# ZpokenWeb3/zk-light-client-implementation

Measured on AMD Instinct MI355X. Metric: Block_i BFT-finality proofs/sec (100 validators), higher is better.
Workload: dtype u64

## Files before the change

### __graft_entry__.py

```python
import os
import subprocess
import sys

ROOT = os.path.dirname(os.path.abspath(__file__))
if ROOT not in sys.path:
    sys.path.insert(0, ROOT)


def build() -> None:
    import concurrent.futures
    import importlib
    b = importlib.import_module("zk-light-client-implementation_amd.build")
    pool = concurrent.futures.ThreadPoolExecutor(max_workers=1)
    devsim = pool.submit(b.build_devsim, True)
    b.build(verbose=True)
    mk = os.path.join(ROOT, "oracle", "c", "Makefile")
    if os.path.exists(mk):
        subprocess.check_call(["make", "-s", "-C", os.path.dirname(mk)])
    import zklc_amd
    zklc_amd.load()
    lib_dir = os.path.join(ROOT, "zk-light-client-implementation_amd", "lib")
    subprocess.check_call(["gcc", "-O2", "-Wall", "-Wextra", "-std=c11", "-D_POSIX_C_SOURCE=200809L", "-I", os.path.join(ROOT, "include"),
                           os.path.join(ROOT, "tests", "c_abi", "prove_from_file.c"), "-o", os.path.join(ROOT, "tests", "c_abi", "prove_from_file"),
                           "-L", lib_dir, "-lzklc_mi355", "-Wl,-rpath,$ORIGIN/../../zk-light-client-implementation_amd/lib"])
    b.build_poseidon_gate_dev(True)
    devsim.result()
    pool.shutdown()


def smoke() -> None:
    import json
    import numpy as np
    import zklc_amd
    from oracle import ed25519_ref as ref

    with zklc_amd.Context(0) as ctx:
        j = json.load(open(os.path.join(ROOT, "tests", "golden", "ed25519_near_c1_small.json")))
        msg = bytes.fromhex(j["msg"])
        pks = b"".join(bytes.fromhex(e["validator_tail"])[1:33] for e in j["entries"])
        sigs = b"".join(bytes.fromhex(e["approval"])[2:] for e in j["entries"])
        ok = ctx.ed25519_verify_batch(pks, sigs, msg)
        exp = [int(ref.verify(pks[32 * i:32 * i + 32], sigs[64 * i:64 * i + 64], msg)) for i in range(len(ok))]
        assert ok.tolist() == exp == [1, 1, 1], (ok.tolist(), exp)
        m2 = b"zklc smoke"
        pk2, sg2, exp2 = [], [], []
        for i in range(64):
            sd = ref.synthetic_seed(11, i)
            _, _, pk = ref.keypair(sd)
            s = bytearray(ref.sign(sd, m2))
            if i % 5 == 4:
                s[i % 64] ^= 0x10
            pk2.append(pk)
            sg2.append(bytes(s))
            exp2.append(int(ref.verify(pk, bytes(s), m2)))
        ok2 = ctx.ed25519_verify_batch(b"".join(pk2), b"".join(sg2), m2)
        assert ok2.tolist() == exp2, "GPU Ed25519 batch differs from the oracle"
        assert sum(exp2) == 64 - 12
        from zklc_amd.plonky2 import CircuitBuilder, serialization as S, HASH_GL
        from oracle import plonky2_prover as OP, plonky2_verifier as V
        b = CircuitBuilder()
        x = b.add_virtual_public_input()
        y = b.add_virtual_target()
        z = b.mul(x, y)
        b.split_le(x, 10)
        lo, hi = b.mul_add_u32(x, y, b.constant(77))
        b.register_public_input(lo)
        b.connect(b.sub(b.add(z, b.constant(5)), z), b.constant(5))
        data = b.build()
        wires, pis = data.generate_witness({x: 1000, y: 4000000000})
        prover = data.prover(ctx, HASH_GL)
        raw = prover.prove_bytes(wires, pis)
        common = data.common_data()
        oproof, ovd = OP.prove(common, data.constants, data.sigmas, wires, pis, V.HasherGL)
        assert raw == S.proof_to_bytes(oproof, common, HASH_GL), "GPU plonky2 proof differs from the oracle prover"
        V.verify(json.loads(json.dumps(S.proof_from_bytes(raw, common, HASH_GL))), prover.verifier_data(), common)
        from zklc_amd.plonky2.recursion import RecursionProver
        rp = RecursionProver(ctx, HASH_GL)
        rc, rproof = rp.recursive_proof((common, prover.verifier_data(), raw), None, [7, 8])
        V.verify(json.loads(json.dumps(rproof)), rc.verifier_only, rc.common)
        assert rproof["public_inputs"] == [7, 8]
        bad = bytearray(raw)
        bad[800] ^= 1
        try:
            rp.recursive_proof((common, prover.verifier_data(), bytes(bad)), None, [7, 8])
            raise SystemExit("smoke: a tampered inner proof was accepted by the in-circuit verifier")
        except AssertionError:
            pass
        rp.close()
        prover.close()
    print("smoke OK: Ed25519 batch verify, a plonky2 proof and a recursive proof on cuda:0 match the oracle")


if __name__ == "__main__":
    build()
    if "--smoke" in sys.argv:
        smoke()
```

### zk-light-client-implementation_amd/build.py

```python
import concurrent.futures as cf
import glob
import os
import subprocess
import sys

HERE = os.path.dirname(os.path.abspath(__file__))
CSRC = os.path.join(HERE, "csrc")
BUILD = os.path.join(HERE, "build")
LIBDIR = os.path.join(HERE, "lib")
LIB = os.path.join(LIBDIR, "libzklc_mi355.so")
HIPCC = os.environ.get("HIPCC", "/opt/rocm/bin/hipcc")
FLAGS = ["--offload-arch=gfx950", "-O3", "-std=c++17", "-fPIC", "-fno-gpu-rdc", "-Wall", "-Wno-unused-function"]


def _newest(paths):
    return max((os.path.getmtime(p) for p in paths), default=0.0)


HOST_CXX = os.environ.get("CXX", "g++")
HOST_FLAGS = ["-O3", "-funroll-loops", "-std=c++17", "-fPIC", "-pthread", "-Wall", "-Wno-unused-function", "-Wno-unknown-pragmas"]


def _compile(src, obj, log):
    cmd = ([HIPCC] + FLAGS if src.endswith(".hip") else [HOST_CXX] + HOST_FLAGS) + ["-c", src, "-o", obj]
    r = subprocess.run(cmd, capture_output=True, text=True)
    if r.returncode != 0:
        raise RuntimeError("hipcc failed for %s:\n%s\n%s" % (src, r.stdout, r.stderr))
    if log:
        print("[zklc build] compiled", os.path.basename(src), file=sys.stderr)
    return obj


def build(verbose=True, force=False):
    os.makedirs(BUILD, exist_ok=True)
    os.makedirs(LIBDIR, exist_ok=True)
    srcs = sorted(glob.glob(os.path.join(CSRC, "*.hip")) + glob.glob(os.path.join(CSRC, "*.cpp")))
    hdrs = glob.glob(os.path.join(CSRC, "*.cuh")) + glob.glob(os.path.join(CSRC, "*.h")) + glob.glob(
        os.path.join(CSRC, "*.inc")) + glob.glob(os.path.join(HERE, "..", "include", "*.h"))
    dep_time = _newest(hdrs + [os.path.abspath(__file__)])
    jobs, objs = [], []
    for s in srcs:
        o = os.path.join(BUILD, os.path.basename(s).replace(".", "_") + ".o")
        objs.append(o)
        if force or not os.path.exists(o) or os.path.getmtime(o) < max(os.path.getmtime(s), dep_time):
            jobs.append((s, o))
    if jobs:
        with cf.ThreadPoolExecutor(max_workers=min(len(jobs), os.cpu_count() or 4)) as ex:
            list(ex.map(lambda so: _compile(so[0], so[1], verbose), jobs))
    if jobs or not os.path.exists(LIB) or os.path.getmtime(LIB) < _newest(objs):
        cmd = [HIPCC, "--offload-arch=gfx950", "-shared", "-fPIC", "-pthread", "-o", LIB] + objs
        r = subprocess.run(cmd, capture_output=True, text=True)
        if r.returncode != 0:
            raise RuntimeError("link failed:\n%s\n%s" % (r.stdout, r.stderr))
        if verbose:
            print("[zklc build] linked", LIB, file=sys.stderr)
    return LIB


DEVSIM_DIR = os.path.join(HERE, "..", "tests", "devsim")
DEVSIM_SRC = os.path.join(DEVSIM_DIR, "devsim.hip")
DEVSIM_LIB = os.path.join(DEVSIM_DIR, "libdevsim.so")


def devsim_sources():
    return [DEVSIM_SRC, os.path.abspath(__file__)] + [p for ext in ("*.cuh", "*.h", "*.inc") for p in glob.glob(os.path.join(CSRC, ext))]


def devsim_is_current():
    return os.path.exists(DEVSIM_LIB) and os.path.getmtime(DEVSIM_LIB) >= _newest(devsim_sources())


def build_devsim(verbose=True, force=False):
    if force or not devsim_is_current():
        r = subprocess.run([HIPCC] + FLAGS + ["-shared", DEVSIM_SRC, "-o", DEVSIM_LIB], capture_output=True, text=True)
        if r.returncode != 0:
            raise RuntimeError("hipcc failed for %s:\n%s\n%s" % (DEVSIM_SRC, r.stdout, r.stderr))
        if verbose:
            print("[zklc build] built", DEVSIM_LIB, file=sys.stderr)
    return DEVSIM_LIB


PGD_DIR = os.path.join(HERE, "..", "tests", "poseidon_gate_dev")
PGD_SRC = os.path.join(PGD_DIR, "poseidon_gate_dev.hip")
PGD_LIB = os.path.join(PGD_DIR, "libposeidon_gate_dev.so")


def poseidon_gate_dev_is_current():
    deps = [PGD_SRC, os.path.abspath(__file__)] + [p for ext in ("*.cuh", "*.h", "*.inc") for p in glob.glob(os.path.join(CSRC, ext))]
    return os.path.exists(PGD_LIB) and os.path.getmtime(PGD_LIB) >= _newest(deps)


def build_poseidon_gate_dev(verbose=True, force=False):
    if force or not poseidon_gate_dev_is_current():
        r = subprocess.run([HIPCC] + FLAGS + ["-Wno-inline-asm", "-shared", PGD_SRC, "-o", PGD_LIB], capture_output=True, text=True)
        if r.returncode != 0:
            raise RuntimeError("hipcc failed for %s:\n%s\n%s" % (PGD_SRC, r.stdout, r.stderr))
        if verbose:
            print("[zklc build] built", PGD_LIB, file=sys.stderr)
    return PGD_LIB


if __name__ == "__main__":
    build(force="--force" in sys.argv)
    build_devsim(force="--force" in sys.argv)
    build_poseidon_gate_dev(force="--force" in sys.argv)
```

### zk-light-client-implementation_amd/csrc/plonky2_prover.hip

```cpp
#include <algorithm>
#include <chrono>
#include <stdio.h>
#include <stdlib.h>
#include <new>
#include <vector>
#include <string.h>
#include "plonky2_gates.cuh"
#include "plonky2_host.h"
#include "plonky2_perm_terms.cuh"
#include "zklc_internal.h"

#define P2_THREADS 256

struct p2_challenges {
    u64 beta[P2_MAX_CH], gamma[P2_MAX_CH], alpha[P2_MAX_CH];
};

__global__ void p2_pow_table_kernel(u64 *out, u64 base, u64 n) {
    u64 i = (u64)blockIdx.x * blockDim.x + threadIdx.x;
    if (i < n) out[i] = gl_pow(base, i);
}

__global__ void p2_scale_by_powers_kernel(u64 *data, u64 base, u64 n) {
    u64 j = (u64)blockIdx.x * blockDim.x + threadIdx.x;
    if (j >= n) return;
    u64 *p = data + (size_t)blockIdx.y * n + j;
    *p = gl_mul(*p, gl_pow(base, j));
}

#define P2_SCALE_PER_LANE 8
__global__ void __launch_bounds__(256) p2_scale_by_powers_strided_kernel(u64 *data, u64 base, u64 step, u64 n) {
    const u64 j0 = (u64)blockIdx.x * (256 * P2_SCALE_PER_LANE) + threadIdx.x;
    if (j0 >= n) return;
    u64 *p = data + (size_t)blockIdx.y * n;
    u64 v[P2_SCALE_PER_LANE];
#pragma unroll
    for (int q = 0; q < P2_SCALE_PER_LANE; q++) v[q] = j0 + 256 * q < n ? p[j0 + 256 * q] : 0;
    u64 pw = gl_pow(base, j0);
#pragma unroll
    for (int q = 0; q < P2_SCALE_PER_LANE; q++) {
        if (j0 + 256 * q < n) p[j0 + 256 * q] = gl_mul(v[q], pw);
        if (q + 1 < P2_SCALE_PER_LANE) pw = gl_mul(pw, step);
    }
}

__global__ void p2_ext_powers_kernel(gl2 *out, gl2 z, u64 n) {
    u64 j = (u64)blockIdx.x * blockDim.x + threadIdx.x;
    if (j < n) out[j] = gl2_pow(z, j);
}

__global__ void p2_ext_pow_limbs_kernel(u32 *out, gl2 z, u32 n) {
    u32 j = blockIdx.x * blockDim.x + threadIdx.x;
    if (j >= n) return;
    gl2 v = gl2_pow(z, j);
    gl_limbs22(v.a, out + 12 * (size_t)j);
    gl_limbs22(v.b, out + 12 * (size_t)j + 6);
}

template <bool LEAN>
__global__ void __launch_bounds__(P2_THREADS)
p2_chunk_products_kernel(const u64 *__restrict__ wires, const u64 *__restrict__ sigmas, const u64 *__restrict__ subgroup,
                         const u64 *__restrict__ k_is, u32 n, u32 routed, u32 qdf, u32 nchunks, u64 beta, u64 gamma,
                         u64 *__restrict__ rp) {
    u32 i = blockIdx.x * blockDim.x + threadIdx.x;
    if (i >= n) return;
    u64 x = subgroup[i];
    u64 nums[16], dens[16];
    for (u32 k = 0; k < nchunks; k++) {
        u64 np = 1, dp = 1;
        u32 end = (k + 1) * qdf < routed ? (k + 1) * qdf : routed;
        if constexpr (LEAN) {
            const u64 bx = gl_mul(beta, x);
            for (u32 j = k * qdf; j < end; j += P2_PERM_CHUNK) {
                const u32 cnt = end - j < P2_PERM_CHUNK ? end - j : P2_PERM_CHUNK;
                u64 wv[P2_PERM_CHUNK], sv[P2_PERM_CHUNK], kv[P2_PERM_CHUNK], n8, d8;
#pragma unroll
                for (u32 q = 0; q < P2_PERM_CHUNK; q++) {
                    const u32 jq = q < cnt ? j + q : j;
                    wv[q] = wires[(size_t)jq * n + i];
                    sv[q] = sigmas[(size_t)jq * n + i];
                    kv[q] = k_is[jq];
                }
                p2_perm_chunk_terms(wv, sv, kv, cnt, beta, bx, gamma, n8, d8);
                if (j == k * qdf) {
                    np = n8;
                    dp = d8;
                } else {
                    np = gl_mul(np, n8);
                    dp = gl_mul(dp, d8);
                }
            }
        } else {
// ... 708 lines not shown
}

#define P2_EVAL_SPLIT 8
__global__ void __launch_bounds__(P2_THREADS)
p2_eval_at_ext_kernel(const u64 *__restrict__ coeffs, u32 n, const gl2 *__restrict__ zpow, const u64 *__restrict__ scale,
                      gl2 *__restrict__ partial) {
    __shared__ gl2 sh[P2_THREADS];
    const u64 *c = coeffs + (size_t)blockIdx.x * n;
    u32 slice = (n + P2_EVAL_SPLIT - 1) / P2_EVAL_SPLIT;
    u32 j0 = blockIdx.y * slice, j1 = j0 + slice < n ? j0 + slice : n;
    gl2 acc = gl2_make(0, 0);
    u32 j = j0 + threadIdx.x;
    for (; j + 3 * P2_THREADS < j1; j += 4 * P2_THREADS) {
        u64 c0 = c[j], c1 = c[j + P2_THREADS], c2 = c[j + 2 * P2_THREADS], c3 = c[j + 3 * P2_THREADS];
        gl2 z0 = zpow[j], z1 = zpow[j + P2_THREADS], z2 = zpow[j + 2 * P2_THREADS], z3 = zpow[j + 3 * P2_THREADS];
        if (scale) {
            c0 = gl_mul(c0, scale[j]);
            c1 = gl_mul(c1, scale[j + P2_THREADS]);
            c2 = gl_mul(c2, scale[j + 2 * P2_THREADS]);
            c3 = gl_mul(c3, scale[j + 3 * P2_THREADS]);
        }
        acc = gl2_add(acc, gl2_add(gl2_add(gl2_scale(z0, c0), gl2_scale(z1, c1)), gl2_add(gl2_scale(z2, c2), gl2_scale(z3, c3))));
    }
    for (; j < j1; j += P2_THREADS) {
        u64 cj = c[j];
        if (scale) cj = gl_mul(cj, scale[j]);
        acc = gl2_add(acc, gl2_scale(zpow[j], cj));
    }
    sh[threadIdx.x] = acc;
    __syncthreads();
    for (u32 off = P2_THREADS / 2; off; off >>= 1) {
        if (threadIdx.x < off) sh[threadIdx.x] = gl2_add(sh[threadIdx.x], sh[threadIdx.x + off]);
        __syncthreads();
    }
    if (threadIdx.x == 0) partial[(size_t)blockIdx.x * P2_EVAL_SPLIT + blockIdx.y] = sh[0];
}
__global__ void p2_eval_finish_kernel(const gl2 *__restrict__ partial, u32 n_polys, gl2 *__restrict__ out) {
    u32 b = blockIdx.x * blockDim.x + threadIdx.x;
    if (b >= n_polys) return;
    gl2 acc = partial[(size_t)b * P2_EVAL_SPLIT];
    for (u32 s = 1; s < P2_EVAL_SPLIT; s++) acc = gl2_add(acc, partial[(size_t)b * P2_EVAL_SPLIT + s]);
    out[b] = acc;
}

struct p2_fri_combine_args {
    const u64 *mats[4];
    u32 widths[4];
    u32 lde_bits, nch;
    u64 w_lde;
    gl2 alpha, zeta, g_zeta, y0, y1, alpha_pow_nch;
    gl2 *out;
    const u32 *apow;
    const u64 *xs;
};
__global__ void __launch_bounds__(P2_THREADS) p2_fri_denominators_kernel(const u64 *__restrict__ xs, u32 lde_bits, gl2 zeta, gl2 g_zeta,
                                                                           gl2 *__restrict__ out) {
    const size_t N = (size_t)1 << lde_bits;
    const size_t p0 = ((size_t)blockIdx.x * blockDim.x + threadIdx.x) * P2_FRI_DEN_POINTS;
    if (p0 >= N) return;
    u64 x[P2_FRI_DEN_POINTS];
    gl2 r[P2_FRI_DEN_POINTS];
#pragma unroll
    for (int q = 0; q < P2_FRI_DEN_POINTS; q++) x[q] = p0 + q < N ? xs[p0 + q] : 0;
    p2_fri_den_inverse_norms(x, zeta, g_zeta, r);
#pragma unroll
    for (int q = 0; q < P2_FRI_DEN_POINTS; q++)
        if (p0 + q < N) out[p0 + q] = r[q];
}
template <bool LEAN>
__global__ void __launch_bounds__(P2_THREADS) p2_fri_combine_kernel(p2_fri_combine_args a) {
    const size_t N = (size_t)1 << a.lde_bits;
    size_t p = (size_t)blockIdx.x * blockDim.x + threadIdx.x;
    if (p >= N) return;
    u64 x;
    [[maybe_unused]] gl2 ninv = gl2_make(0, 0);
    if constexpr (LEAN) {
        x = a.xs[p];
        ninv = a.out[p];
    } else {
        u64 i = __brevll((u64)p) >> (64 - a.lde_bits);
        x = gl_mul(GL_GENERATOR, gl_pow(a.w_lde, i));
    }
    gl_acc3 sa = {0, 0, 0}, sb = {0, 0, 0};
    gl_ktab *k6 = (gl_ktab *)a.apow;
    u32 terms = 0;
    for (int m = 0; m < 4; m++) {
        const u64 *mat = a.mats[m] + p;
        const u32 w = a.widths[m];
        u32 j = 0;
        for (; j + 16 <= w; j += 16, k6 += 16 * 12) {
            u64 v[16];
#pragma unroll
            for (int q = 0; q < 16; q++) v[q] = mat[(size_t)(j + q) * N];
#pragma unroll
            for (int q = 0; q < 16; q++) {
                gl_acc3_mul(sa, v[q], k6 + 12 * q);
                gl_acc3_mul(sb, v[q], k6 + 12 * q + 6);
            }
            if ((terms += 16) >= 384) {
                terms = 0;
                gl_acc3_normalize(sa);
                gl_acc3_normalize(sb);
            }
        }
        for (; j < w; j++, k6 += 12) {
            u64 v = mat[(size_t)j * N];
            gl_acc3_mul(sa, v, k6);
            gl_acc3_mul(sb, v, k6 + 6);
        }
        terms += 16;
    }
    gl2 acc = gl2_make(gl_acc3_reduce(sa), gl_acc3_reduce(sb));
    gl_acc3 ta = {0, 0, 0}, tb = {0, 0, 0};
    for (u32 j = 0; j < a.nch; j++) {
        u64 v = a.mats[2][(size_t)j * N + p];
        gl_acc3_mul(ta, v, (gl_ktab *)a.apow + 12 * (size_t)j);
        gl_acc3_mul(tb, v, (gl_ktab *)a.apow + 12 * (size_t)j + 6);
    }
    gl2 acc1 = gl2_make(gl_acc3_reduce(ta), gl_acc3_reduce(tb));
    gl2 i0, i1;
    if constexpr (LEAN) {
        i0 = p2_fri_den_inverse(x, a.zeta, ninv.a);
        i1 = p2_fri_den_inverse(x, a.g_zeta, ninv.b);
    } else {
        i0 = gl2_inv(gl2_sub(gl2_make(x, 0), a.zeta));
        i1 = gl2_inv(gl2_sub(gl2_make(x, 0), a.g_zeta));
    }
    gl2 q0 = gl2_mul(gl2_sub(acc, a.y0), i0);
    gl2 q1 = gl2_mul(gl2_sub(acc1, a.y1), i1);
    a.out[p] = gl2_add(gl2_mul(q0, a.alpha_pow_nch), q1);
}

__global__ void __launch_bounds__(P2_THREADS)
p2_fri_fold_kernel(const gl2 *__restrict__ in, gl2 *__restrict__ out, u32 log_m, u32 a_bits, u64 shift, u64 w_m, u64 w_a_inv,
                   u64 a_inv, gl2 beta) {
    __shared__ u64 tw[64];
    const u32 A = 1u << a_bits;
    if (threadIdx.x < A) tw[threadIdx.x] = gl_pow(w_a_inv, threadIdx.x);
    __syncthreads();
    u32 chunks = 1u << (log_m - a_bits);
    u32 l = blockIdx.x * blockDim.x + threadIdx.x;
    if (l >= chunks) return;
    u32 m = log_m == a_bits ? 0 : (u32)(__brevll((u64)l) >> (64 - (log_m - a_bits)));
    u64 x = gl_mul(shift, gl_pow(w_m, m));
    gl2 r = gl2_scale(beta, gl_inv(x));
    const gl2 *v = in + (size_t)l * A;
    gl2 acc = gl2_make(0, 0);
    for (u32 i = A; i-- > 0;) {
        gl2 c = gl2_make(0, 0);
        for (u32 e = 0; e < A; e++) {
            u32 j = __brev(e) >> (32 - a_bits);
            c = gl2_add(c, gl2_scale(v[e], tw[(i * j) & (A - 1)]));
        }
        acc = gl2_add(gl2_mul(acc, r), c);
    }
    out[l] = gl2_scale(acc, a_inv);
}

__global__ void __launch_bounds__(P2_THREADS)
p2_fri_final_poly_kernel(const gl2 *__restrict__ in, gl2 *__restrict__ out, u32 log_m, u64 shift_inv, u64 w_m_inv, u64 m_inv) {
    u32 M = 1u << log_m;
    u32 k = blockIdx.x * blockDim.x + threadIdx.x;
    if (k >= M) return;
    u64 wk = gl_pow(w_m_inv, k);
    gl2 acc = gl2_make(0, 0);
    u64 t = 1;
    for (u32 i = 0; i < M; i++) {
        u32 pos = log_m ? (u32)(__brevll((u64)i) >> (64 - log_m)) : 0;
        acc = gl2_add(acc, gl2_scale(in[pos], t));
        t = gl_mul(t, wk);
    }
    out[k] = gl2_scale(acc, gl_mul(m_inv, gl_pow(shift_inv, k)));
}

struct p2_pow_args {
    u64 state[12];
    u64 in[8];
    u32 n_in, pow_bits;
    u64 base;
    unsigned long long *found;
};
template <bool TAIL>
__global__ void __launch_bounds__(P2_THREADS) p2_pow_kernel(p2_pow_args a) {
    u64 w = a.base + (u64)blockIdx.x * blockDim.x + threadIdx.x;
    if (TAIL && __hip_atomic_load(a.found, __ATOMIC_RELAXED, __HIP_MEMORY_SCOPE_AGENT) < w) return;
    u64 s[12];
#pragma unroll
    for (int i = 0; i < 12; i++) s[i] = a.state[i];
#pragma unroll
    for (int i = 0; i < 8; i++)
        if ((u32)i < a.n_in) s[i] = a.in[i];
#pragma unroll
    for (int i = 0; i < 8; i++)
        if ((u32)i == a.n_in) s[i] = w;
    if (TAIL) poseidon_gl_permute_keep<4>(s);
    else poseidon_gl_permute(s);
    if ((s[7] >> (64 - a.pow_bits)) == 0) atomicMin(a.found, (unsigned long long)w);
}

struct p2_gather {
    const u64 *src;
    u64 stride;
    u32 count, dst;
};
__global__ void p2_gather_kernel(const p2_gather *__restrict__ d, u32 nd, u64 *__restrict__ out) {
    u32 g = blockIdx.x;
    if (g >= nd) return;
    p2_gather e = d[g];
    for (u32 i = threadIdx.x; i < e.count; i += blockDim.x) out[e.dst + i] = e.src[(size_t)i * e.stride];
}

static u64 h_mul(u64 a, u64 b) { return (u64)(((unsigned __int128)a * b) % GL_P); }
static u64 h_add(u64 a, u64 b) { return (u64)(((unsigned __int128)a + b) % GL_P); }
static u64 h_sub(u64 a, u64 b) { return a >= b ? a - b : a + GL_P - b; }
static u64 h_pow(u64 a, u64 e) {
    u64 r = 1;
    while (e) {
        if (e & 1) r = h_mul(r, a);
        a = h_mul(a, a);
        e >>= 1;
    }
    return r;
}
static u64 h_inv(u64 a) { return h_pow(a, GL_P - 2); }
static u64 h_root(u32 log_n) { return h_pow(GL_POWER_OF_TWO_GENERATOR, 1ULL << (32 - log_n)); }
static gl2 h2_mul(gl2 x, gl2 y) {
    return gl2_make(h_add(h_mul(x.a, y.a), h_mul(7, h_mul(x.b, y.b))), h_add(h_mul(x.a, y.b), h_mul(x.b, y.a)));
}
static gl2 h2_add(gl2 x, gl2 y) { return gl2_make(h_add(x.a, y.a), h_add(x.b, y.b)); }
static gl2 h2_pow(gl2 x, u64 e) {
    gl2 r = gl2_make(1, 0);
    while (e) {
        if (e & 1) r = h2_mul(r, x);
        x = h2_mul(x, x);
        e >>= 1;
    }
    return r;
}

struct p2_batch {
    u32 width = 0;
    u64 *coeffs = nullptr, *lde = nullptr, *tree = nullptr;
};

struct zklc_plonky2_circuit {
    zklc_ctx *ctx = nullptr;
    int device = 0;
    zklc_plonky2_params P;
    u32 n = 0, N = 0, lde_bits = 0, nchunks = 0;
    std::vector<p2_gate> gates;
    p2_gate *d_gates = nullptr;
    u64 *d_extra = nullptr, *d_kis = nullptr, *d_subgroup = nullptr, *d_sigma_vals = nullptr;
    p2_batch cs, wires, zs, quot;
    u64 *d_wire_vals = nullptr;
    u64 *d_rp = nullptr, *d_excl = nullptr, *d_totals = nullptr, *d_grand = nullptr;
    u64 *d_qv = nullptr;
    u32 *d_apow = nullptr;
    u32 *d_fri_apow = nullptr;
    u64 *d_xs = nullptr, *d_l0 = nullptr;
    p2_fused_plan plan = {};
    size_t fused_lds = 0;
    std::vector<double> gate_ms;
    gl2 *d_zpow = nullptr, *d_open = nullptr, *d_open_partial = nullptr;
    gl2 *d_fri[9] = {};
    u64 *d_fri_tree[8] = {};
    gl2 *d_final = nullptr;
    unsigned long long *d_found = nullptr;
    p2_gather *d_gather = nullptr;
    u64 *d_gather_out = nullptr;
    size_t gather_cap = 0, gather_out_words = 0;
    std::vector<uint8_t> cap_bytes;
    uint8_t digest[32];
    std::vector<u64> last_challenges;
    double timings[8] = {};
    u64 tree_words = 0;
    std::vector<void *> allocs;
    std::vector<std::pair<uint8_t *, size_t>> pin_blocks;
    size_t pin_used = 0;
};

static bool p2_pin_enabled() {
    static const bool on = !(getenv("ZKLC_PINNED_STAGING") && getenv("ZKLC_PINNED_STAGING")[0] == '0');
    return on;
}
static void p2_pin_free(void *q) {
    if (p2_pin_enabled()) (void)hipHostFree(q);
    else free(q);
}
static void *p2_pin(zklc_plonky2_circuit *c, size_t bytes) {
    bytes = (bytes + 63) & ~(size_t)63;
    if (c->pin_blocks.empty() || c->pin_used + bytes > c->pin_blocks.back().second) {
        size_t cap = bytes > (1u << 20) ? bytes : (1u << 20);
        void *q = nullptr;
        if (!p2_pin_enabled()) {
            q = malloc(cap);
            if (!q) return nullptr;
        } else if (hipHostMalloc(&q, cap, hipHostMallocDefault) != hipSuccess) {
            (void)hipGetLastError();
            return nullptr;
        }
        c->pin_blocks.push_back({(uint8_t *)q, cap});
        c->pin_used = 0;
    }
    void *r = c->pin_blocks.back().first + c->pin_used;
    c->pin_used += bytes;
    return r;
}
static void p2_pin_reset(zklc_plonky2_circuit *c) {
    if (c->pin_blocks.size() > 1) {
        size_t total = 0;
        for (auto &b : c->pin_blocks) {
            total += b.second;
            p2_pin_free(b.first);
        }
        c->pin_blocks.clear();
        void *q = nullptr;
        if (!p2_pin_enabled()) {
            if ((q = malloc(total))) c->pin_blocks.push_back({(uint8_t *)q, total});
        } else if (hipHostMalloc(&q, total, hipHostMallocDefault) == hipSuccess) c->pin_blocks.push_back({(uint8_t *)q, total});
        else (void)hipGetLastError();
    }
    c->pin_used = 0;
}
#define P2_PIN(c, ptr, type, count)                                          \
    type *ptr = (type *)p2_pin((c), sizeof(type) * (size_t)(count));          \
    if (!ptr) {                                                               \
        (c)->ctx->last_err = "hipHostMalloc: pinned staging";                 \
        return ZKLC_ERR_OOM;                                                  \
    }

static int32_t p2_alloc(zklc_plonky2_circuit *c, void **p, size_t bytes) {
    zklc_ctx *ctx = c->ctx;
    ZKLC_HIP(ctx, hipMalloc(p, bytes ? bytes : 8));
    c->allocs.push_back(*p);
    return ZKLC_OK;
}
#define P2_ALLOC(c, ptr, bytes)                                      \
    do {                                                             \
        int32_t rc__ = p2_alloc((c), (void **)&(ptr), (bytes));      \
        if (rc__) return rc__;                                       \
    } while (0)
#define P2_RC(call)               \
    do {                          \
        int32_t rc__ = (call);    \
        if (rc__) return rc__;    \
    } while (0)

static inline u64 *p2_tree_level(u64 *tree, u32 log_leaves, u32 level) {
    u64 off = 0;
    for (u32 j = 0; j < level; j++) off += 4ULL << (log_leaves - j);
    return tree + off;
}

static int32_t p2_merkle(zklc_plonky2_circuit *c, hipStream_t st, const u64 *mat, u64 stride, u64 leaf_stride, u32 log_leaves,
                         u32 width, u64 *tree) {
    u32 cap_h = c->P.cap_height < log_leaves ? c->P.cap_height : log_leaves;
    if (c->P.hasher == ZKLC_HASHER_POSEIDON_GL)
        return zklc_gl_merkle_commit_strided(c->ctx, st, mat, stride, leaf_stride, log_leaves, width, cap_h, tree);
    return zklc_bn254_merkle_commit_strided(c->ctx, st, mat, stride, leaf_stride, log_leaves, width, cap_h, tree);
}

static int32_t p2_commit_coeffs(zklc_plonky2_circuit *c, hipStream_t st, p2_batch &b, std::vector<uint8_t> &cap) {
    zklc_ctx *ctx = c->ctx;
    P2_RC(zklc_gl_lde_dev(ctx, st, b.coeffs, c->P.degree_bits, c->P.rate_bits, b.width, GL_GENERATOR, b.lde, ZKLC_NTT_OUT_BITREV));
    P2_RC(p2_merkle(c, st, b.lde, c->N, 1, c->lde_bits, b.width, b.tree));
    u32 cap_h = c->P.cap_height < c->lde_bits ? c->P.cap_height : c->lde_bits;
    cap.resize((size_t)32 << cap_h);
    P2_PIN(c, h_cap, uint8_t, cap.size());
    ZKLC_HIP(ctx, zklc_readback_async(h_cap, p2_tree_level(b.tree, c->lde_bits, c->lde_bits - cap_h), cap.size(), st));
    ZKLC_HIP(ctx, zklc_stream_wait(st));
    memcpy(cap.data(), h_cap, cap.size());
    return ZKLC_OK;
}
static int32_t p2_commit_values(zklc_plonky2_circuit *c, hipStream_t st, p2_batch &b, std::vector<uint8_t> &cap) {
    P2_RC(zklc_gl_ntt_dev(c->ctx, st, b.coeffs, c->P.degree_bits, b.width, ZKLC_NTT_INVERSE, 0));
    return p2_commit_coeffs(c, st, b, cap);
}

static int32_t p2_hash_no_pad(zklc_plonky2_circuit *c, hipStream_t st, const std::vector<u64> &v, uint8_t *out32) {
    zklc_ctx *ctx = c->ctx;
    if (c->P.hasher == ZKLC_HASHER_POSEIDON_GL) {
        u64 h[4];
        zklc_host_poseidon_hash_no_pad(v.data(), v.size(), h);
        memcpy(out32, h, 32);
        return ZKLC_OK;
    }
    if (v.size() <= 3) return ZKLC_ERR_INVALID_ARG;
    void *d;
    P2_RC(zklc_stage(ctx, 6, v.size() * 8 + 64, &d));
    u64 *dv = (u64 *)d;
    P2_PIN(c, h_v, u64, v.size() + 4);
    memcpy(h_v + 4, v.data(), v.size() * 8);
    ZKLC_HIP(ctx, hipMemcpyAsync(dv + 8, h_v + 4, v.size() * 8, hipMemcpyHostToDevice, st));
    P2_RC(zklc_bn254_merkle_commit_strided(ctx, st, dv + 8, 1, 0, 0, (u32)v.size(), 0, dv));
    ZKLC_HIP(ctx, zklc_readback_async(h_v, dv, 32, st));
    ZKLC_HIP(ctx, zklc_stream_wait(st));
    memcpy(out32, h_v, 32);
    return ZKLC_OK;
}

static void p2_quotient_static_args(const zklc_plonky2_circuit *c, p2_quotient_args &a) {
    const zklc_plonky2_params &P = c->P;
    a.cs = c->cs.lde;
    a.wires = c->wires.lde;
    a.zs = c->zs.lde;
    a.gates = c->d_gates;
    a.extra = c->d_extra;
    a.k_is = c->d_kis;
    a.lde_bits = c->lde_bits;
    a.degree_bits = P.degree_bits;
    a.rate_bits = P.rate_bits;
    a.num_constants = P.num_constants;
// ... 89 lines not shown

extern "C" void zklc_plonky2_circuit_destroy(zklc_plonky2_circuit *c) {
    if (!c) return;
    (void)hipSetDevice(c->device);
    (void)hipDeviceSynchronize();
    for (void *p : c->allocs) (void)hipFree(p);
    for (auto &b : c->pin_blocks) p2_pin_free(b.first);
    delete c;
}

static int32_t p2_create(zklc_ctx *ctx, const zklc_plonky2_params *params, const zklc_plonky2_gate *gates, const uint64_t *gate_extra,
                         uint32_t gate_extra_words, const uint64_t *k_is, const uint64_t *constants, const uint64_t *sigmas,
                         zklc_plonky2_circuit *c) {
    const zklc_plonky2_params &P = *params;
    c->ctx = ctx;
    c->device = ctx->device;
    c->P = P;
    c->n = 1u << P.degree_bits;
    c->lde_bits = P.degree_bits + P.rate_bits;
    c->N = 1u << c->lde_bits;
    c->nchunks = P.num_partial_products + 1;
    const u32 n = c->n, N = c->N;
    hipStream_t st = ctx->stream;
    ZKLC_HIP(ctx, hipSetDevice(ctx->device));
    c->gates.resize(P.num_gates);
    for (u32 i = 0; i < P.num_gates; i++) {
        p2_gate g;
        g.type = gates[i].type;
        for (int k = 0; k < 4; k++) g.p[k] = gates[i].p[k];
        g.selector_index = gates[i].selector_index;
        g.group_start = gates[i].group_start;
        g.group_end = gates[i].group_end;
        g.extra_off = gates[i].extra_off;
        if (g.type >= P2_NUM_GATE_TYPES || g.selector_index >= P.num_selectors) return ZKLC_ERR_INVALID_ARG;
        if (g.type == P2_RANDOM_ACCESS && g.p[0] > 6) return ZKLC_ERR_INVALID_ARG;
        if (g.type == P2_COSET_INTERPOLATION && (g.p[0] > 5 || g.p[1] < 2 || g.extra_off + (2u << g.p[0]) > gate_extra_words))
            return ZKLC_ERR_INVALID_ARG;
        c->gates[i] = g;
    }
    P2_ALLOC(c, c->d_gates, sizeof(p2_gate) * P.num_gates);
    ZKLC_HIP(ctx, hipMemcpyAsync(c->d_gates, c->gates.data(), sizeof(p2_gate) * P.num_gates, hipMemcpyHostToDevice, st));
    P2_ALLOC(c, c->d_extra, (size_t)gate_extra_words * 8);
    if (gate_extra_words) ZKLC_HIP(ctx, hipMemcpyAsync(c->d_extra, gate_extra, (size_t)gate_extra_words * 8, hipMemcpyHostToDevice, st));
    P2_ALLOC(c, c->d_kis, (size_t)P.num_routed_wires * 8);
    ZKLC_HIP(ctx, hipMemcpyAsync(c->d_kis, k_is, (size_t)P.num_routed_wires * 8, hipMemcpyHostToDevice, st));
    const u32 nch_ = P.num_challenges;
    P2_ALLOC(c, c->d_subgroup, (size_t)n * 8);
    hipLaunchKernelGGL(p2_pow_table_kernel, dim3((n + 255) / 256), dim3(256), 0, st, c->d_subgroup, h_root(P.degree_bits), (u64)n);
    ZKLC_HIP(ctx, hipGetLastError());

    c->tree_words = zklc_gl_merkle_tree_words(c->lde_bits, P.cap_height < c->lde_bits ? P.cap_height : c->lde_bits);
    auto alloc_batch = [&](p2_batch &b, u32 width) -> int32_t {
        b.width = width;
        P2_ALLOC(c, b.coeffs, (size_t)width * n * 8);
        P2_ALLOC(c, b.lde, (size_t)width * N * 8);
        P2_ALLOC(c, b.tree, c->tree_words * 8);
        return ZKLC_OK;
    };
    const u32 nch = P.num_challenges;
    P2_RC(alloc_batch(c->cs, P.num_constants + P.num_routed_wires));
    P2_RC(alloc_batch(c->wires, P.num_wires));
    P2_RC(alloc_batch(c->zs, nch * (1 + P.num_partial_products)));
    c->quot.width = nch * P.quotient_degree_factor;
    P2_ALLOC(c, c->d_qv, (size_t)nch * N * 8);
    c->quot.coeffs = c->d_qv;
    P2_ALLOC(c, c->quot.lde, (size_t)c->quot.width * N * 8);
    P2_ALLOC(c, c->quot.tree, c->tree_words * 8);
    P2_ALLOC(c, c->d_wire_vals, (size_t)P.num_wires * n * 8);
    P2_ALLOC(c, c->d_sigma_vals, (size_t)P.num_routed_wires * n * 8);
    P2_ALLOC(c, c->d_rp, (size_t)c->nchunks * n * 8);
    P2_ALLOC(c, c->d_excl, (size_t)n * 8);
    P2_ALLOC(c, c->d_totals, (size_t)((n + P2_SCAN_BLOCK - 1) / P2_SCAN_BLOCK) * 8);
    P2_ALLOC(c, c->d_grand, 8);
    P2_ALLOC(c, c->d_apow, (size_t)nch_ * (nch_ + nch_ * (P.num_partial_products + 1) + P.num_gate_constraints + 1) * 24);
    P2_ALLOC(c, c->d_zpow, (size_t)n * sizeof(gl2));
    P2_ALLOC(c, c->d_fri_apow, (size_t)(c->cs.width + c->wires.width + c->zs.width + c->quot.width + 1) * 12 * sizeof(u32));
    P2_ALLOC(c, c->d_xs, (size_t)N * 8);
    P2_ALLOC(c, c->d_l0, (size_t)N * 8);
    u32 total_polys = c->cs.width + c->wires.width + c->zs.width + c->quot.width + nch;
    P2_ALLOC(c, c->d_open, (size_t)total_polys * sizeof(gl2));
    P2_ALLOC(c, c->d_open_partial, (size_t)total_polys * P2_EVAL_SPLIT * sizeof(gl2));
    u32 bits = c->lde_bits;
    P2_ALLOC(c, c->d_fri[0], (size_t)N * sizeof(gl2));
    for (u32 r = 0; r < P.num_arities; r++) {
        u32 leaves_bits = bits - P.arity_bits[r];
        u32 cap_h = P.cap_height < leaves_bits ? P.cap_height : leaves_bits;
        P2_ALLOC(c, c->d_fri_tree[r], zklc_gl_merkle_tree_words(leaves_bits, cap_h) * 8);
        bits = leaves_bits;
        P2_ALLOC(c, c->d_fri[r + 1], ((size_t)1 << bits) * sizeof(gl2));
    }
    P2_ALLOC(c, c->d_final, ((size_t)1 << bits) * sizeof(gl2));
    P2_ALLOC(c, c->d_found, 8);

    size_t cbytes = (size_t)P.num_constants * n * 8, sbytes = (size_t)P.num_routed_wires * n * 8;
    ZKLC_HIP(ctx, hipMemcpyAsync(c->cs.coeffs, constants, cbytes, hipMemcpyHostToDevice, st));
    ZKLC_HIP(ctx, hipMemcpyAsync(c->cs.coeffs + (size_t)P.num_constants * n, sigmas, sbytes, hipMemcpyHostToDevice, st));
    ZKLC_HIP(ctx, hipMemcpyAsync(c->d_sigma_vals, sigmas, sbytes, hipMemcpyHostToDevice, st));
    P2_RC(p2_commit_values(c, st, c->cs, c->cap_bytes));
    {
        p2_quotient_args a = {};
        p2_quotient_static_args(c, a);
        hipLaunchKernelGGL(p2_point_tables_kernel, dim3((N / 4 + 255) / 256 ? (N / 4 + 255) / 256 : 1), dim3(256), 0, st, c->d_xs, c->d_l0,
                           c->lde_bits, P.rate_bits, a.w_lde, a.n_field, a);
        ZKLC_HIP(ctx, hipGetLastError());
        P2_RC(p2_plan_quotient(c, st));
    }

    auto hash_to_vec = [&](const uint8_t *h, std::vector<u64> &out) {
        if (P.hasher == ZKLC_HASHER_POSEIDON_GL) {
            u64 v[4];
            memcpy(v, h, 32);
            out.insert(out.end(), v, v + 4);
        } else {
            for (int off = 0; off < 32; off += 7) {
                u64 v = 0;
                memcpy(&v, h + off, 32 - off < 7 ? 32 - off : 7);
                out.push_back(v);
            }
        }
    };
    std::vector<u64> parts;
    for (size_t i = 0; i < c->cap_bytes.size(); i += 32) hash_to_vec(c->cap_bytes.data() + i, parts);
    std::vector<u64> pad;
    pad.push_back(1);
    u32 pad_to = P.hasher == ZKLC_HASHER_POSEIDON_GL ? 8 : 9;
    while ((pad.size() + 1) % pad_to) pad.push_back(0);
    pad.push_back(1);
    uint8_t dsep[32];
    P2_RC(p2_hash_no_pad(c, st, pad, dsep));
    hash_to_vec(dsep, parts);
    parts.push_back(P.degree_bits);
    P2_RC(p2_hash_no_pad(c, st, parts, c->digest));
    return ZKLC_OK;
}

extern "C" int32_t zklc_plonky2_circuit_create(zklc_ctx *ctx, const zklc_plonky2_params *params, const zklc_plonky2_gate *gates,
                                               const uint64_t *gate_extra, uint32_t gate_extra_words, const uint64_t *k_is,
                                               const uint64_t *constants, const uint64_t *sigmas, zklc_plonky2_circuit **out) {
    if (!ctx || !params || !gates || !k_is || !constants || !sigmas || !out) return ZKLC_ERR_INVALID_ARG;
    const zklc_plonky2_params &P = *params;
    if (P.num_challenges == 0 || P.num_challenges > P2_MAX_CH || P.degree_bits == 0 || P.degree_bits + P.rate_bits > ZKLC_GL_MAX_LOG ||
        P.rate_bits > 4 || P.quotient_degree_factor != (1u << P.rate_bits) || P.num_arities > 8 || P.hasher > 1 ||
        P.num_routed_wires > P.num_wires || P.num_selectors == 0 || P.num_selectors > P.num_constants || P.num_gates == 0 ||
        P.num_partial_products + 1 > 16 || (P.num_partial_products + 1) * P.quotient_degree_factor < P.num_routed_wires ||
        P.proof_of_work_bits == 0 || P.proof_of_work_bits > 40)
        return ZKLC_ERR_INVALID_ARG;
    u32 bits = P.degree_bits + P.rate_bits;
    for (u32 r = 0; r < P.num_arities; r++) {
        if (P.arity_bits[r] == 0 || P.arity_bits[r] > 5 || P.arity_bits[r] > bits) return ZKLC_ERR_INVALID_ARG;
        bits -= P.arity_bits[r];
    }
    if (bits < P.rate_bits) return ZKLC_ERR_INVALID_ARG;
    zklc_plonky2_circuit *c = new (std::nothrow) zklc_plonky2_circuit();
    if (!c) return ZKLC_ERR_OOM;
    int32_t rc = p2_create(ctx, params, gates, gate_extra, gate_extra_words, k_is, constants, sigmas, c);
    if (rc) {
        zklc_plonky2_circuit_destroy(c);
        return rc;
    }
    *out = c;
    return ZKLC_OK;
}

extern "C" int32_t zklc_plonky2_verifier_data(zklc_plonky2_circuit *c, uint8_t *cap_out, uint8_t *digest_out) {
    if (!c || !cap_out || !digest_out) return ZKLC_ERR_INVALID_ARG;
    memcpy(cap_out, c->cap_bytes.data(), c->cap_bytes.size());
// ... 201 lines not shown
        }
        ZKLC_HIP(ctx, hipGetLastError());
        P2_RC(zklc_gl_ntt_dev(ctx, st, c->d_qv, c->lde_bits, nch, ZKLC_NTT_INVERSE | ZKLC_NTT_IN_BITREV, 0));
        if (zklc_lean_arith()) {
            const u64 gi = h_inv(GL_GENERATOR);
            hipLaunchKernelGGL(p2_scale_by_powers_strided_kernel, dim3((N + 256 * P2_SCALE_PER_LANE - 1) / (256 * P2_SCALE_PER_LANE), nch),
                               dim3(256), 0, st, c->d_qv, gi, h_pow(gi, 256), (u64)N);
        } else {
            hipLaunchKernelGGL(p2_scale_by_powers_kernel, dim3((N + 255) / 256, nch), dim3(256), 0, st, c->d_qv, h_inv(GL_GENERATOR), (u64)N);
        }
        ZKLC_HIP(ctx, hipGetLastError());
        P2_RC(p2_commit_coeffs(c, st, c->quot, quot_cap));
    }
    p2_observe_cap(ch, quot_cap, hasher);
    gl2 zeta;
    zeta.a = ch.challenge();
    zeta.b = ch.challenge();
    lap(2);

    const u32 w0 = c->cs.width, w1 = c->wires.width, w2 = c->zs.width, w3 = c->quot.width;
    const u32 n_open = w0 + w1 + w2 + w3 + nch;
    P2_PIN(c, open, gl2, n_open);
    {
        hipLaunchKernelGGL(p2_ext_powers_kernel, dim3((n + 255) / 256), dim3(256), 0, st, c->d_zpow, zeta, (u64)n);
        const p2_batch *bs[4] = {&c->cs, &c->wires, &c->zs, &c->quot};
        u32 off = 0;
        for (int k = 0; k < 4; k++) {
            hipLaunchKernelGGL(p2_eval_at_ext_kernel, dim3(bs[k]->width, P2_EVAL_SPLIT), dim3(P2_THREADS), 0, st,
                               (const u64 *)bs[k]->coeffs, n, (const gl2 *)c->d_zpow, (const u64 *)nullptr,
                               c->d_open_partial + (size_t)off * P2_EVAL_SPLIT);
            off += bs[k]->width;
        }
        hipLaunchKernelGGL(p2_eval_at_ext_kernel, dim3(nch, P2_EVAL_SPLIT), dim3(P2_THREADS), 0, st, (const u64 *)c->zs.coeffs, n,
                           (const gl2 *)c->d_zpow, (const u64 *)c->d_subgroup, c->d_open_partial + (size_t)off * P2_EVAL_SPLIT);
        hipLaunchKernelGGL(p2_eval_finish_kernel, dim3((n_open + 255) / 256), dim3(256), 0, st, (const gl2 *)c->d_open_partial, n_open,
                           c->d_open);
        ZKLC_HIP(ctx, hipGetLastError());
        ZKLC_HIP(ctx, zklc_readback_async(open, c->d_open, (size_t)n_open * sizeof(gl2), st));
        ZKLC_HIP(ctx, zklc_stream_wait(st));
    }
    for (u32 i = 0; i < n_open; i++) {
        ch.observe(open[i].a);
        ch.observe(open[i].b);
    }
    gl2 fri_alpha;
    fri_alpha.a = ch.challenge();
    fri_alpha.b = ch.challenge();
    lap(3);

    std::vector<std::vector<uint8_t>> fri_caps(P.num_arities);
    std::vector<gl2> fri_betas(P.num_arities);
    u32 final_bits;
    {
        p2_fri_combine_args a = {};
        a.mats[0] = c->cs.lde;
        a.mats[1] = c->wires.lde;
        a.mats[2] = c->zs.lde;
        a.mats[3] = c->quot.lde;
        a.widths[0] = w0;
        a.widths[1] = w1;
        a.widths[2] = w2;
        a.widths[3] = w3;
        a.lde_bits = c->lde_bits;
        a.nch = nch;
        a.w_lde = h_root(c->lde_bits);
        a.alpha = fri_alpha;
        a.zeta = zeta;
        a.g_zeta = gl2_make(h_mul(zeta.a, h_root(P.degree_bits)), h_mul(zeta.b, h_root(P.degree_bits)));
        gl2 y0 = gl2_make(0, 0), y1 = gl2_make(0, 0);
        for (u32 i = w0 + w1 + w2 + w3; i-- > 0;) y0 = h2_add(h2_mul(y0, fri_alpha), open[i]);
        for (u32 i = nch; i-- > 0;) y1 = h2_add(h2_mul(y1, fri_alpha), open[w0 + w1 + w2 + w3 + i]);
        a.y0 = y0;
        a.y1 = y1;
        a.alpha_pow_nch = h2_pow(fri_alpha, nch);
        a.out = c->d_fri[0];
        a.apow = c->d_fri_apow;
        hipLaunchKernelGGL(p2_ext_pow_limbs_kernel, dim3((w0 + w1 + w2 + w3 + 255) / 256), dim3(256), 0, st, c->d_fri_apow, fri_alpha,
                           w0 + w1 + w2 + w3);
        a.xs = c->d_xs;
        if (zklc_lean_arith()) {
            const u32 lanes = (N + P2_FRI_DEN_POINTS - 1) / P2_FRI_DEN_POINTS;
            hipLaunchKernelGGL(p2_fri_denominators_kernel, dim3((lanes + P2_THREADS - 1) / P2_THREADS), dim3(P2_THREADS), 0, st,
                               (const u64 *)c->d_xs, c->lde_bits, a.zeta, a.g_zeta, a.out);
            hipLaunchKernelGGL(p2_fri_combine_kernel<true>, dim3((N + P2_THREADS - 1) / P2_THREADS), dim3(P2_THREADS), 0, st, a);
        } else {
            hipLaunchKernelGGL(p2_fri_combine_kernel<false>, dim3((N + P2_THREADS - 1) / P2_THREADS), dim3(P2_THREADS), 0, st, a);
        }
        ZKLC_HIP(ctx, hipGetLastError());
        u32 bits = c->lde_bits;
        u64 shift = GL_GENERATOR;
        for (u32 r = 0; r < P.num_arities; r++) {
            u32 ab = P.arity_bits[r], A = 1u << ab;
            u32 leaves_bits = bits - ab;
            P2_RC(p2_merkle(c, st, (const u64 *)c->d_fri[r], 1, 2 * A, leaves_bits, 2 * A, c->d_fri_tree[r]));
            u32 cap_h = P.cap_height < leaves_bits ? P.cap_height : leaves_bits;
            fri_caps[r].resize((size_t)32 << cap_h);
            P2_PIN(c, h_fcap, uint8_t, fri_caps[r].size());
            ZKLC_HIP(ctx, zklc_readback_async(h_fcap, p2_tree_level(c->d_fri_tree[r], leaves_bits, leaves_bits - cap_h), fri_caps[r].size(), st));
            ZKLC_HIP(ctx, zklc_stream_wait(st));
            memcpy(fri_caps[r].data(), h_fcap, fri_caps[r].size());
            p2_observe_cap(ch, fri_caps[r], hasher);
            fri_betas[r].a = ch.challenge();
            fri_betas[r].b = ch.challenge();
            u32 chunks = 1u << leaves_bits;
            hipLaunchKernelGGL(p2_fri_fold_kernel, dim3((chunks + P2_THREADS - 1) / P2_THREADS), dim3(P2_THREADS), 0, st,
                               (const gl2 *)c->d_fri[r], c->d_fri[r + 1], bits, ab, shift, h_root(bits), h_inv(h_root(ab)),
                               h_inv(A), fri_betas[r]);
            ZKLC_HIP(ctx, hipGetLastError());
            shift = h_pow(shift, A);
            bits = leaves_bits;
        }
        final_bits = bits;
        u32 M = 1u << bits;
        hipLaunchKernelGGL(p2_fri_final_poly_kernel, dim3((M + P2_THREADS - 1) / P2_THREADS), dim3(P2_THREADS), 0, st,
                           (const gl2 *)c->d_fri[P.num_arities], c->d_final, bits, h_inv(shift), h_inv(h_root(bits)), h_inv(M));
        ZKLC_HIP(ctx, hipGetLastError());
    }
    const size_t final_n = (size_t)1 << final_bits;
    P2_PIN(c, final_poly, gl2, final_n);
    ZKLC_HIP(ctx, zklc_readback_async(final_poly, c->d_final, final_n * sizeof(gl2), st));
    ZKLC_HIP(ctx, zklc_stream_wait(st));
    const u32 final_len = 1u << (final_bits - P.rate_bits);
    for (size_t i = final_len; i < final_n; i++)
        if (final_poly[i].a || final_poly[i].b) {
            ctx->last_err = "plonky2: FRI final polynomial has a non-zero high coefficient (witness does not satisfy the circuit)";
            return ZKLC_ERR_INVALID_ARG;
        }
    for (u32 i = 0; i < final_len; i++) {
        ch.observe(final_poly[i].a);
        ch.observe(final_poly[i].b);
    }
    lap(4);

    u64 pow_witness;
    {
        p2_pow_args a = {};
        for (int i = 0; i < 12; i++) a.state[i] = ch.state[i];
        for (int i = 0; i < ch.n_in; i++) a.in[i] = ch.in[i];
        a.n_in = ch.n_in;
        a.pow_bits = P.proof_of_work_bits;
        a.found = c->d_found;
        const u32 batch_bits = P.proof_of_work_bits + 2 < 24 ? P.proof_of_work_bits + 2 : 24;
        const u64 batch = (1ULL << batch_bits) > P2_THREADS ? 1ULL << batch_bits : P2_THREADS;
        P2_PIN(c, h_found, unsigned long long, 1);
        unsigned long long found = ~0ULL;
        for (u64 base = 0;; base += batch) {
            ZKLC_HIP(ctx, hipMemsetAsync(c->d_found, 0xFF, 8, st));
            a.base = base;
            hipLaunchKernelGGL(zklc_pgl_tail() ? p2_pow_kernel<true> : p2_pow_kernel<false>, dim3((unsigned)(batch / P2_THREADS)),
                               dim3(P2_THREADS), 0, st, a);
            ZKLC_HIP(ctx, hipGetLastError());
            ZKLC_HIP(ctx, zklc_readback_async(h_found, c->d_found, 8, st));
            ZKLC_HIP(ctx, zklc_stream_wait(st));
            found = *h_found;
            if (found != ~0ULL) break;
            if (base > (1ULL << 50)) return ZKLC_ERR_INVALID_ARG;
        }
        pow_witness = found;
        ch.observe(pow_witness);
        u64 resp = ch.challenge();
        if (resp >> (64 - P.proof_of_work_bits)) {
            ctx->last_err = "plonky2: proof-of-work response mismatch between the kernel and the host transcript";
            return ZKLC_ERR_HIP;
        }
    }
    lap(5);

// ... 144 lines not shown
```

Baseline: 0.2243.

## Combine FRI polynomials in coefficient form before LDE instead of per LDE point

When lean arithmetic is on, the alpha-weighted FRI combination now runs over the n polynomial coefficients instead of the N LDE points. It produces four combined base-field columns, extends them with a single 4-column LDE, and a finish kernel then applies the quotient denominators per point. This replaces a reduction over every committed column at rate-expanded size with one over coefficients, at the cost of an extra NTT, two more buffers, and one more launch. An environment variable restores the per-point path.

```diff
diff --git a/__graft_entry__.py b/__graft_entry__.py
--- a/__graft_entry__.py
+++ b/__graft_entry__.py
@@ -24,6 +24,7 @@
                            os.path.join(ROOT, "tests", "c_abi", "prove_from_file.c"), "-o", os.path.join(ROOT, "tests", "c_abi", "prove_from_file"),
                            "-L", lib_dir, "-lzklc_mi355", "-Wl,-rpath,$ORIGIN/../../zk-light-client-implementation_amd/lib"])
     b.build_poseidon_gate_dev(True)
+    b.build_fri_coeff_dev(True)
     devsim.result()
     pool.shutdown()
 
diff --git a/zk-light-client-implementation_amd/build.py b/zk-light-client-implementation_amd/build.py
--- a/zk-light-client-implementation_amd/build.py
+++ b/zk-light-client-implementation_amd/build.py
@@ -100,7 +100,34 @@
     return PGD_LIB
 
 
+FCD_DIR = os.path.join(HERE, "..", "tests", "fri_coeff_dev")
+FCD_SRC = os.path.join(FCD_DIR, "fri_coeff_dev.hip")
+FCD_CASES = os.path.join(FCD_DIR, "fri_coeff_dev_cases.cpp")
+FCD_LIB = os.path.join(FCD_DIR, "libfri_coeff_dev.so")
+
+
+def fri_coeff_dev_is_current():
+    deps = [FCD_SRC, FCD_CASES, os.path.join(HERE, "..", "tests", "fri_coeff_host", "fri_coeff_cases.h"), os.path.abspath(__file__)]
+    deps += [p for ext in ("*.cuh", "*.h", "*.inc") for p in glob.glob(os.path.join(CSRC, ext))]
+    return os.path.exists(FCD_LIB) and os.path.getmtime(FCD_LIB) >= _newest(deps)
+
+
+def build_fri_coeff_dev(verbose=True, force=False):
+    if force or not fri_coeff_dev_is_current():
+        obj, kobj = os.path.join(FCD_DIR, "fri_coeff_dev_cases.o"), os.path.join(FCD_DIR, "fri_coeff_dev.o")
+        for cmd in ([HOST_CXX, "-O2", "-std=c++17", "-fPIC", "-Wall", "-Wno-unused-function", "-Wno-unknown-pragmas", "-c", FCD_CASES, "-o", obj],
+                    [HIPCC] + FLAGS + ["-c", FCD_SRC, "-o", kobj],
+                    [HIPCC, "--offload-arch=gfx950", "-shared", "-fPIC", "-o", FCD_LIB, kobj, obj]):
+            r = subprocess.run(cmd, capture_output=True, text=True)
+            if r.returncode != 0:
+                raise RuntimeError("%s failed for %s:\n%s\n%s" % (cmd[0], FCD_DIR, r.stdout[-4000:], r.stderr[-4000:]))
+        if verbose:
+            print("[zklc build] built", FCD_LIB, file=sys.stderr)
+    return FCD_LIB
+
+
 if __name__ == "__main__":
     build(force="--force" in sys.argv)
     build_devsim(force="--force" in sys.argv)
     build_poseidon_gate_dev(force="--force" in sys.argv)
+    build_fri_coeff_dev(force="--force" in sys.argv)
diff --git a/zk-light-client-implementation_amd/csrc/plonky2_fri_combine.cuh b/zk-light-client-implementation_amd/csrc/plonky2_fri_combine.cuh
--- /dev/null
+++ b/zk-light-client-implementation_amd/csrc/plonky2_fri_combine.cuh
@@ -0,0 +1,93 @@
+#pragma once
+#include "plonky2_perm_terms.cuh"
+
+#define P2_FRI_THREADS 256
+
+ZKLC_HD void p2_fri_alpha_sum(const u64 *const (&mats)[4], const u32 (&widths)[4], size_t stride, size_t p, gl_ktab *k6, gl_acc3 &sa,
+                              gl_acc3 &sb) {
+    u32 terms = 0;
+    for (int m = 0; m < 4; m++) {
+        const u64 *mat = mats[m] + p;
+        const u32 w = widths[m];
+        u32 j = 0;
+        for (; j + 16 <= w; j += 16, k6 += 16 * 12) {
+            u64 v[16];
+#if defined(__HIP_DEVICE_COMPILE__)
+#pragma unroll
+#endif
+            for (int q = 0; q < 16; q++) v[q] = mat[(size_t)(j + q) * stride];
+#if defined(__HIP_DEVICE_COMPILE__)
+#pragma unroll
+#endif
+            for (int q = 0; q < 16; q++) {
+                gl_acc3_mul(sa, v[q], k6 + 12 * q);
+                gl_acc3_mul(sb, v[q], k6 + 12 * q + 6);
+            }
+            if ((terms += 16) >= 384) {
+                terms = 0;
+                gl_acc3_normalize(sa);
+                gl_acc3_normalize(sb);
+            }
+        }
+        for (; j < w; j++, k6 += 12) {
+            u64 v = mat[(size_t)j * stride];
+            gl_acc3_mul(sa, v, k6);
+            gl_acc3_mul(sb, v, k6 + 6);
+        }
+        terms += 16;
+    }
+}
+ZKLC_HD gl2 p2_fri_zs_sum(const u64 *zs, u32 nch, size_t stride, size_t p, gl_ktab *k6) {
+    gl_acc3 ta = {0, 0, 0}, tb = {0, 0, 0};
+    for (u32 j = 0; j < nch; j++) {
+        u64 v = zs[(size_t)j * stride + p];
+        gl_acc3_mul(ta, v, k6 + 12 * (size_t)j);
+        gl_acc3_mul(tb, v, k6 + 12 * (size_t)j + 6);
+    }
+    return gl2_make(gl_acc3_reduce(ta), gl_acc3_reduce(tb));
+}
+
+struct p2_fri_coeff_args {
+    const u64 *coeffs[4];
+    u32 widths[4];
+    u32 n, nch;
+    const u32 *apow;
+    u64 *out;
+};
+ZKLC_HD void p2_fri_coeff_lane(const p2_fri_coeff_args &a, size_t j) {
+    gl_acc3 sa = {0, 0, 0}, sb = {0, 0, 0};
+    p2_fri_alpha_sum(a.coeffs, a.widths, a.n, j, (gl_ktab *)a.apow, sa, sb);
+    const gl2 h = p2_fri_zs_sum(a.coeffs[2], a.nch, a.n, j, (gl_ktab *)a.apow);
+    a.out[j] = gl_acc3_reduce(sa);
+    a.out[(size_t)a.n + j] = gl_acc3_reduce(sb);
+    a.out[2 * (size_t)a.n + j] = h.a;
+    a.out[3 * (size_t)a.n + j] = h.b;
+}
+
+struct p2_fri_finish_args {
+    const u64 *gh;
+    const u64 *xs;
+    u32 lde_bits;
+    gl2 zeta, g_zeta, y0, y1, alpha_pow_nch;
+    gl2 *out;
+};
+ZKLC_HD void p2_fri_finish_lane(const p2_fri_finish_args &a, size_t p) {
+    const size_t N = (size_t)1 << a.lde_bits;
+    const u64 x = a.xs[p];
+    const gl2 ninv = a.out[p];
+    const gl2 g = gl2_make(a.gh[p], a.gh[N + p]), h = gl2_make(a.gh[2 * N + p], a.gh[3 * N + p]);
+    const gl2 q0 = gl2_mul(gl2_sub(g, a.y0), p2_fri_den_inverse(x, a.zeta, ninv.a));
+    const gl2 q1 = gl2_mul(gl2_sub(h, a.y1), p2_fri_den_inverse(x, a.g_zeta, ninv.b));
+    a.out[p] = gl2_add(gl2_mul(q0, a.alpha_pow_nch), q1);
+}
+
+#if defined(__HIPCC__)
+__global__ void __launch_bounds__(P2_FRI_THREADS) p2_fri_coeff_combine_kernel(p2_fri_coeff_args a) {
+    const size_t j = (size_t)blockIdx.x * blockDim.x + threadIdx.x;
+    if (j < a.n) p2_fri_coeff_lane(a, j);
+}
+__global__ void __launch_bounds__(P2_FRI_THREADS) p2_fri_coeff_finish_kernel(p2_fri_finish_args a) {
+    const size_t p = (size_t)blockIdx.x * blockDim.x + threadIdx.x;
+    if (p < ((size_t)1 << a.lde_bits)) p2_fri_finish_lane(a, p);
+}
+#endif
diff --git a/zk-light-client-implementation_amd/csrc/plonky2_prover.hip b/zk-light-client-implementation_amd/csrc/plonky2_prover.hip
--- a/zk-light-client-implementation_amd/csrc/plonky2_prover.hip
+++ b/zk-light-client-implementation_amd/csrc/plonky2_prover.hip
@@ -8,6 +8,7 @@
 #include "plonky2_gates.cuh"
 #include "plonky2_host.h"
 #include "plonky2_perm_terms.cuh"
+#include "plonky2_fri_combine.cuh"
 #include "zklc_internal.h"
 
 #define P2_THREADS 256
@@ -882,42 +883,9 @@
         x = gl_mul(GL_GENERATOR, gl_pow(a.w_lde, i));
     }
     gl_acc3 sa = {0, 0, 0}, sb = {0, 0, 0};
-    gl_ktab *k6 = (gl_ktab *)a.apow;
-    u32 terms = 0;
-    for (int m = 0; m < 4; m++) {
-        const u64 *mat = a.mats[m] + p;
-        const u32 w = a.widths[m];
-        u32 j = 0;
-        for (; j + 16 <= w; j += 16, k6 += 16 * 12) {
-            u64 v[16];
-#pragma unroll
-            for (int q = 0; q < 16; q++) v[q] = mat[(size_t)(j + q) * N];
-#pragma unroll
-            for (int q = 0; q < 16; q++) {
-                gl_acc3_mul(sa, v[q], k6 + 12 * q);
-                gl_acc3_mul(sb, v[q], k6 + 12 * q + 6);
-            }
-            if ((terms += 16) >= 384) {
-                terms = 0;
-                gl_acc3_normalize(sa);
-                gl_acc3_normalize(sb);
-            }
-        }
-        for (; j < w; j++, k6 += 12) {
-            u64 v = mat[(size_t)j * N];
-            gl_acc3_mul(sa, v, k6);
-            gl_acc3_mul(sb, v, k6 + 6);
-        }
-        terms += 16;
-    }
+    p2_fri_alpha_sum(a.mats, a.widths, N, p, (gl_ktab *)a.apow, sa, sb);
     gl2 acc = gl2_make(gl_acc3_reduce(sa), gl_acc3_reduce(sb));
-    gl_acc3 ta = {0, 0, 0}, tb = {0, 0, 0};
-    for (u32 j = 0; j < a.nch; j++) {
-        u64 v = a.mats[2][(size_t)j * N + p];
-        gl_acc3_mul(ta, v, (gl_ktab *)a.apow + 12 * (size_t)j);
-        gl_acc3_mul(tb, v, (gl_ktab *)a.apow + 12 * (size_t)j + 6);
-    }
-    gl2 acc1 = gl2_make(gl_acc3_reduce(ta), gl_acc3_reduce(tb));
+    gl2 acc1 = p2_fri_zs_sum(a.mats[2], a.nch, N, p, (gl_ktab *)a.apow);
     gl2 i0, i1;
     if constexpr (LEAN) {
         i0 = p2_fri_den_inverse(x, a.zeta, ninv.a);
@@ -1063,6 +1031,7 @@
     std::vector<double> gate_ms;
     gl2 *d_zpow = nullptr, *d_open = nullptr, *d_open_partial = nullptr;
     gl2 *d_fri[9] = {};
+    u64 *d_fri_gh = nullptr, *d_fri_gh_lde = nullptr;
     u64 *d_fri_tree[8] = {};
     gl2 *d_final = nullptr;
     unsigned long long *d_found = nullptr;
@@ -1128,6 +1097,11 @@
         (c)->ctx->last_err = "hipHostMalloc: pinned staging";                 \
         return ZKLC_ERR_OOM;                                                  \
     }
+
+static bool p2_fri_combine_on_coeffs() {
+    static const bool on = zklc_lean_arith() && !(getenv("ZKLC_P2_FRI_COMBINE") && !strcmp(getenv("ZKLC_P2_FRI_COMBINE"), "points"));
+    return on;
+}
 
 static int32_t p2_alloc(zklc_plonky2_circuit *c, void **p, size_t bytes) {
     zklc_ctx *ctx = c->ctx;
@@ -1383,6 +1357,12 @@
     P2_ALLOC(c, c->d_open_partial, (size_t)total_polys * P2_EVAL_SPLIT * sizeof(gl2));
     u32 bits = c->lde_bits;
     P2_ALLOC(c, c->d_fri[0], (size_t)N * sizeof(gl2));
+    if (p2_fri_combine_on_coeffs()) {
+        P2_ALLOC(c, c->d_fri_gh, (size_t)4 * n * 8);
+        P2_ALLOC(c, c->d_fri_gh_lde, (size_t)4 * N * 8);
+    }
+    if (getenv("ZKLC_P2_DEBUG"))
+        fprintf(stderr, "[zklc] fri combine: %s\n", p2_fri_combine_on_coeffs() ? "coefficients" : zklc_lean_arith() ? "points" : "points, as it was");
     for (u32 r = 0; r < P.num_arities; r++) {
         u32 leaves_bits = bits - P.arity_bits[r];
         u32 cap_h = P.cap_height < leaves_bits ? P.cap_height : leaves_bits;
@@ -1750,7 +1730,34 @@
             const u32 lanes = (N + P2_FRI_DEN_POINTS - 1) / P2_FRI_DEN_POINTS;
             hipLaunchKernelGGL(p2_fri_denominators_kernel, dim3((lanes + P2_THREADS - 1) / P2_THREADS), dim3(P2_THREADS), 0, st,
                                (const u64 *)c->d_xs, c->lde_bits, a.zeta, a.g_zeta, a.out);
-            hipLaunchKernelGGL(p2_fri_combine_kernel<true>, dim3((N + P2_THREADS - 1) / P2_THREADS), dim3(P2_THREADS), 0, st, a);
+            if (p2_fri_combine_on_coeffs()) {
+                p2_fri_coeff_args ca = {};
+                const p2_batch *bs[4] = {&c->cs, &c->wires, &c->zs, &c->quot};
+                for (int k = 0; k < 4; k++) {
+                    ca.coeffs[k] = bs[k]->coeffs;
+                    ca.widths[k] = bs[k]->width;
+                }
+                ca.n = n;
+                ca.nch = nch;
+                ca.apow = c->d_fri_apow;
+                ca.out = c->d_fri_gh;
+                hipLaunchKernelGGL(p2_fri_coeff_combine_kernel, dim3((n + P2_FRI_THREADS - 1) / P2_FRI_THREADS), dim3(P2_FRI_THREADS), 0, st, ca);
+                ZKLC_HIP(ctx, hipGetLastError());
+                P2_RC(zklc_gl_lde_dev(ctx, st, c->d_fri_gh, P.degree_bits, P.rate_bits, 4, GL_GENERATOR, c->d_fri_gh_lde, ZKLC_NTT_OUT_BITREV));
+                p2_fri_finish_args fa = {};
+                fa.gh = c->d_fri_gh_lde;
+                fa.xs = c->d_xs;
+                fa.lde_bits = c->lde_bits;
+                fa.zeta = a.zeta;
+                fa.g_zeta = a.g_zeta;
+                fa.y0 = a.y0;
+                fa.y1 = a.y1;
+                fa.alpha_pow_nch = a.alpha_pow_nch;
+                fa.out = a.out;
+                hipLaunchKernelGGL(p2_fri_coeff_finish_kernel, dim3((N + P2_FRI_THREADS - 1) / P2_FRI_THREADS), dim3(P2_FRI_THREADS), 0, st, fa);
+            } else {
+                hipLaunchKernelGGL(p2_fri_combine_kernel<true>, dim3((N + P2_THREADS - 1) / P2_THREADS), dim3(P2_THREADS), 0, st, a);
+            }
         } else {
             hipLaunchKernelGGL(p2_fri_combine_kernel<false>, dim3((N + P2_THREADS - 1) / P2_THREADS), dim3(P2_THREADS), 0, st, a);
         }
```

Measured after the change: 0.2274, median of 6. 1.01x the previous value.
